# SamsungSAILMontreal/ghn3

Measured on AMD Instinct MI355X. Metric: predicted-params/sec (GHN fwd+bwd), ghn3xlm16, 256-node graphs, higher is better.
Workload: dtype f16; 1 GPU; ghn3xlm16 fwd+bwd, 1 synthetic 256-node graph(s) per GPU (seed 256000+), 86515016 predicted params per GPU, loss = sum of Frobenius norms of the predicted tensors; ghn_params=654365312, decoder_rows=1421, workspace_bytes=2436048640, zero_fill_bytes=2797339192, parallelism=dp1, index_mode=reference, loss=fused into the tile kernels

## Files before the change

ghn3_amd/build.py:

```python
import os
import subprocess
import sys
from concurrent.futures import ThreadPoolExecutor

HERE = os.path.dirname(os.path.abspath(__file__))
ROOT = os.path.dirname(HERE)
CSRC = os.path.join(HERE, 'csrc')
OUT_DIR = os.path.join(HERE, 'lib')
LIB = os.path.join(OUT_DIR, 'libghn3_hip.so')
SOURCES = ['gemm.hip', 'gemm_p8.hip', 'gemm_small.hip', 'gemm_x3.hip', 'gemm_x3d.hip', 'gemm_wg.hip', 'attention.hip', 'elementwise.hip', 'target_ops.hip', 'tnet_msa.hip', 'tnet_attn.hip', 'tnet_head.hip', 'tnet_wgrad.hip', 'tnet_join.hip', 'runtime.hip']
FLAGS = ['--offload-arch=gfx950', '-O3', '-std=c++17', '-fPIC', '-I' + os.path.join(ROOT, 'include'),
         '-I' + CSRC, '-Wno-unused-result'] + os.environ.get('GHN3_HIPCC_EXTRA', '').split()


def _hipcc():
    for cand in (os.environ.get('HIPCC'), '/opt/rocm/bin/hipcc', 'hipcc'):
        if cand and (os.path.isabs(cand) and os.path.exists(cand) or not os.path.isabs(cand)):
            return cand
    raise RuntimeError('hipcc not found')


def _stale(target, deps):
    if not os.path.exists(target):
        return True
    t = os.path.getmtime(target)
    return any(os.path.getmtime(d) > t for d in deps)


def source_hash():
    import hashlib
    h = hashlib.sha256()
    files = [os.path.join(CSRC, f) for f in sorted(os.listdir(CSRC)) if f.endswith(('.hip', '.h'))]
    files += [os.path.join(ROOT, 'include', 'ghn3_hip.h'), os.path.join(HERE, 'program.py')]
    for f in files:
        with open(f, 'rb') as fh:
            h.update(os.path.basename(f).encode() + b'\0' + fh.read())
    return h.hexdigest()[:16]


def build(force=False, verbose=True):
    os.makedirs(OUT_DIR, exist_ok=True)
    hipcc = _hipcc()
    headers = [os.path.join(ROOT, 'include', 'ghn3_hip.h'), os.path.join(CSRC, 'ghn3_internal.h'),
# ... 27 lines not shown
```

ghn3_amd/csrc/ghn3_internal.h:

```cpp
#pragma once
#include <hip/hip_runtime.h>
#include <stdint.h>
#include "ghn3_hip.h"

struct GemmProbDev {
    const float* A; const float* B; float* C;
    const float* bias; const float* residual; const float* aux_in; float* aux_out;
    const int* a_gather; const int* b_gather; const int* c_gather;
    int M, N, K, lda, ldb, ldc;
    int a_q, a_s, b_q, b_s, c_q, c_s;
    int bias_q, bias_s, bias_stride;
    int act, dact, flags;
    float alpha;
    int tile_start;
    int tiles_m, tiles_n;
    int ksplit, k_chunk;
    int order;
    int kq, ks;
    const int* lim;
    int lim_kind;
    int xcd_cols;
    int pin;
    int pin_first, pin_count;
    int pin_end, pin_total;
    const float* alpha_amax;
    int ln_kind;
    float ln_eps;
    const float* ln_p[6];
    const void* B2;
    const int* mtab;
};


int ghn3_gemm_init();
int ghn3_gemm_launch(const GemmProbDev* d_probs, int n_probs, int total_tiles, int a_mode, int b_mode,
                     int tile, int ctype, hipStream_t stream);

int ghn3_gemm_h16d_launch(const GemmProbDev* d_probs, int n_probs, int total_tiles, int tile, int ctype, int grid_cap,
                          hipStream_t stream);
int ghn3_gemm_p8_init();
int ghn3_gemm_p8_launch(const GemmProbDev* d_probs, int n_probs, int total_tiles, int ctype, int grid_cap,
                        hipStream_t stream);
int ghn3_gemm_p8w_launch(const GemmProbDev* d_probs, int n_probs, int total_tiles, int ctype, int grid_cap,
                         hipStream_t stream);
int ghn3_gemm_p8d_launch(const GemmProbDev* d_probs, int n_probs, int total_tiles, int ctype, int grid_cap,
                         hipStream_t stream);
int ghn3_gemm_x3_init();
int ghn3_gemm_x3_tile(int code, int slice, int* bm, int* bn);
int ghn3_gemm_x3_launch(const GemmProbDev* d_probs, int n_probs, int total_tiles, int code, int slice,
                        hipStream_t stream);
int ghn3_gemm_x3s_init();
int ghn3_gemm_x3s_tile(int code, int K, int ln_kind, int* bm, int* bn);
int ghn3_gemm_x3s_launch(const GemmProbDev* d_probs, const GemmProbDev* h_probs, int n_probs, int total_tiles, int code, int K,
                         int ln_kind, hipStream_t stream);
int ghn3_gemm_wg_launch(const GemmProbDev* d_probs, int n_probs, int total_tiles, int grid_cap, int tile_edge, hipStream_t stream);
int ghn3_gemm_small_launch(const GemmProbDev* d_probs, int n_probs, int total_tiles, int a_mode, int b_mode, int with_ln,
                           hipStream_t stream);

int ghn3_attn_init();
int ghn3_attn_fwd(float* out, const float* qkv, const float* bias, float* P, const int* n_nodes,
                  int B, int N, int C, int H, hipStream_t s);
int ghn3_attn_bwd(float* dqkv, const float* dO, const float* qkv, const float* P, const float* O, float* amax_out,
                  float* dBias, const int* n_nodes, int B, int N, int C, int H, int general, hipStream_t s);

int ghn3_graph_prologue(const int64_t* A, int* deg_in, int* deg_out, int* dist0, int* pair,
                        int B, int N, int V, hipStream_t s);
int ghn3_embed_nodes(float* x, const int* node_type, const int* shape_idx, const int* n_nodes, const int* node_off,
                     const float* E_type, const float* E_ch, const float* E_sp, const float* E_in,
                     const float* E_out, const float* E_dist, const int* deg_in, const int* deg_out,
                     const int* dist0, int B, int N, int C, hipStream_t s);
int ghn3_embed_bwd(const float* dx, const int* node_type, const int* shape_idx, const int* n_nodes,
                   const int* node_off, float* dE_type, float* dE_ch, float* dE_sp, float* dE_in, float* dE_out,
                   float* dE_dist, const int* deg_in, const int* deg_out, const int* dist0,
                   int B, int N, int C, int n_type, int n_ch, int n_sp, hipStream_t s);
int ghn3_edge_hidden(float* hid, const float* Pfw, const float* Pbw, int V, int C, hipStream_t s);
int ghn3_edge_hidden_bwd(float* dPfw, float* dPbw, float* dhid, const float* hid, int V, int C, hipStream_t s);
int ghn3_bias_gather(float* bias, const float* T, const int* pair, int B, int N, int H, hipStream_t s);
int ghn3_bias_hist(float* dT, const float* dBias, const int* pair, int B, int N, int H, int V, void* scratch,
                   int have_amax, hipStream_t s);
int ghn3_rowset_colsum(float* out, const float* X, const void* sets, int n_sets, int O, int I, hipStream_t s);
int ghn3_layernorm_fwd(float* y, float* x, const float* g, const float* b, float* mean, float* rstd, const float* add,
                       int n_add, int64_t add_stride, int rows, int C, float eps, hipStream_t s);
int ghn3_layernorm_bwd(float* dx, float* dy, const float* x, const float* g, const float* mean,
                       const float* rstd, const float* res, const float* add, int n_add, int64_t add_stride, int rows,
                       int C, hipStream_t s);
int ghn3_ln_param_grad(float* dg, float* db, const float* dy, const float* x, const float* mean,
                       const float* rstd, int rows, int C, int accum, hipStream_t s);
int ghn3_ln_param_grad_batch(float* gbase, const float* abase, const int64_t* table, int n_items, int rows, int C,
// ... 62 lines not shown
```

ghn3_amd/csrc/runtime.hip:

```cpp

#include "ghn3_internal.h"
#include <cstdarg>
#include <cstdio>
#include <cstring>
#include <vector>
#include <algorithm>

static thread_local char g_err[512] = "";

void ghn3_set_error(const char* fmt, ...) {
    va_list ap;
    va_start(ap, fmt);
    vsnprintf(g_err, sizeof(g_err), fmt, ap);
    va_end(ap);
}

extern "C" const char* ghn3_last_error(void) { return g_err; }
extern "C" int ghn3_abi_version(void) { return GHN3_ABI_VERSION; }

#define HIPCHK(expr)                                                                  \
    do {                                                                              \
        hipError_t e_ = (expr);                                                       \
        if (e_ != hipSuccess) {                                                       \
            ghn3_set_error("%s failed: %s", #expr, hipGetErrorString(e_));            \
// ... 161 lines not shown
        if (ms256) ms256[i] = c->tag_ms[i];
        if (n256) n256[i] = c->tag_n[i];
        if (reset) { c->tag_ms[i] = 0; c->tag_n[i] = 0; }
    }
    return GHN3_OK;
}

struct Resolver {
    void* const* bufs; int n_bufs; bool bad;
    template <typename T> T* get(const ghn3_ref& r) {
        if (r.buf < 0) return nullptr;
        if (r.buf >= n_bufs || bufs[r.buf] == nullptr) { bad = true; return nullptr; }
        return reinterpret_cast<T*>(reinterpret_cast<char*>(bufs[r.buf]) + r.off);
    }
};

static int pick_tile(const ghn3_gemm_problem& p, int forced, int64_t op_t64) {
    if (p.flags & GHN3_GEMM_X3) {
        if (forced == 44 || forced == 45 || p.ln_kind)
            return (forced == 45 ? 7000 : 6000) + 100 * (p.ln_kind & 3) + ((p.K / 64) % 100);
        return 4000 + 10 * (((forced >= 40 && forced <= 42) ? forced : 40) - 40) + p.x3_slice / 64;
    }
    if (p.ln_kind) return 32;
    if (p.flags & GHN3_GEMM_OP16) {
        if (forced == 16 || forced == 24 || forced == 20 || forced == 25 || forced == 29 || forced == 30) return forced;
        if (forced == 28) {
            const bool kmap_ok = p.b_kq == 0 || p.b_kq % 64 == 0 || 64 % p.b_kq == 0;
            return (p.ksplit <= 1 && p.M >= 160 && (p.N & 3) == 0 && kmap_ok && p.a_gather.buf < 0 && p.b_gather.buf < 0 &&
                    p.c_gather.buf < 0) ? 28 : 16;
        }
        const int64_t t256 = (int64_t)((p.M + 255) / 256) * ((p.N + 255) / 256) * (p.ksplit > 1 ? p.ksplit : 1);
        const double eff = ((double)p.M / (((p.M + 255) / 256) * 256.0)) * ((double)p.N / (((p.N + 255) / 256) * 256.0));
        return (t256 >= 200 && eff >= 0.8) ? 24 : 16;
    }
    if (forced == 48 || forced == 49) {
        const bool ok = p.a_mode == GHN3_MODE_COL && p.b_mode == GHN3_MODE_COL && p.ksplit <= 1 && (p.M & 3) == 0 &&
                        (p.N & 3) == 0 && (p.ldc & 3) == 0 && (p.C.off & 15) == 0 && (p.lda & 3) == 0 && (p.ldb & 3) == 0 &&
                        (p.A.off & 15) == 0 && (p.B.off & 15) == 0 && p.a_gather.buf < 0 &&
                        p.b_gather.buf < 0 && p.c_gather.buf < 0 && !p.a_q && !p.b_q && !p.c_q && !p.bias_q &&
                        p.act == GHN3_ACT_NONE && p.dact == GHN3_DACT_NONE && p.residual.buf < 0 && p.aux_out.buf < 0 &&
                        (p.bias.buf < 0 || (p.flags & GHN3_GEMM_BIASGRAD));
        return ok ? forced : 64;
    }
    if (forced == 32 || forced == 64 || forced == 128) return forced;
    const double flops = 2.0 * p.M * p.N * (double)p.K;
    if (p.ksplit <= 1 && op_t64 <= 640 && flops <= 4e9 && p.K <= 8192) return 32;
    const int64_t t128 = (int64_t)((p.M + 127) / 128) * ((p.N + 127) / 128) * (p.ksplit > 1 ? p.ksplit : 1);
    if (p.M >= 96 && p.N >= 96 && t128 >= 192) return 128;
    return 64;
}

static inline bool is16(int tl) { return tl == 16 || tl == 24 || tl == 20 || tl == 25 || tl == 28 || tl == 29 || tl == 30; }

extern "C" int ghn3_run(ghn3_ctx* c, const ghn3_op* ops, int n_ops, const ghn3_gemm_problem* problems, int n_problems,
                        void* const* bufs, int n_bufs, void* stream_) {
    if (!c) return GHN3_E_NOCTX;
    if (n_ops < 0 || (n_ops > 0 && !ops) || n_bufs < 0) { ghn3_set_error("ghn3_run: bad arguments"); return GHN3_E_ARG; }
    hipStream_t stream = (hipStream_t)stream_;
    Resolver R{bufs, n_bufs, false};

    std::vector<std::vector<Launch>> fresh_launches;
    const std::vector<std::vector<Launch>>* launches = &fresh_launches;
    size_t need = 0;
    for (int k = 0; k < n_ops; ++k)
        if (ops[k].kind == GHN3_OP_GEMM) need += (size_t)ops[k].i[1];
    GemmProbDev* hs = nullptr; GemmProbDev* ds = nullptr;
// ... 24 lines not shown
        for (int i = 1; i < kStageSlots; ++i)
            if (c->cache[i].stamp < c->cache[slot].stamp) slot = i;
        c->cache[slot].valid = false;
        c->cache_misses++;
        if (c->ev_used[slot]) { HIPCHK(hipEventSynchronize(c->ev[slot])); c->ev_used[slot] = false; }
        hs = c->h_stage[slot]; ds = c->d_stage[slot];
        std::vector<std::vector<Launch>>& op_launches = fresh_launches;
        op_launches.resize(n_ops);
        size_t pos = 0;
        for (int k = 0; k < n_ops; ++k) {
            if (ops[k].kind != GHN3_OP_GEMM) continue;
            const int first = (int)ops[k].i[0], cnt = (int)ops[k].i[1], forced = (int)ops[k].i[2];
            if (first < 0 || cnt < 0 || first + cnt > n_problems) {
                ghn3_set_error("op %d: GEMM problem range [%d,%d) outside table of %d", k, first, first + cnt, n_problems);
                return GHN3_E_ARG;
            }
            int64_t op_t64 = 0;
            for (int q = first; q < first + cnt; ++q)
                op_t64 += (int64_t)((problems[q].M + 63) / 64) * ((problems[q].N + 63) / 64);
            std::vector<int> codes;
            for (int q = first; q < first + cnt; ++q) {
                if (problems[q].M <= 0 || problems[q].N <= 0) continue;
                const int tc = pick_tile(problems[q], forced, op_t64);
                if (std::find(codes.begin(), codes.end(), tc) == codes.end()) codes.push_back(tc);
            }
            std::sort(codes.begin(), codes.end());
            for (int am = 0; am < 2; ++am)
                for (int bm = 0; bm < 2; ++bm)
                    for (int tl : codes) {
                        Launch L{am, bm, tl, (int)pos, 0, 0, 0, 0};
                        int te = tl == 16 ? 128 : (tl == 24 || tl == 20 || tl == 25 || tl == 28 || tl == 29 || tl == 30) ? 256 : tl == 48 ? 64 : tl == 49 ? 128 : tl;
                        int te_n = (tl == 20 || tl == 30) ? 128 : te;
                        const bool x3 = tl >= 4000;
                        const bool x3old = x3 && tl < 5000;
                        if (x3old && !ghn3_gemm_x3_tile(40 + (tl - 4000) / 10, 64 * (tl % 10), &te, &te_n)) {
                            ghn3_set_error("op %d: no split-bf16 kernel for tile bucket %d (tile code %d, K slice %d)", k, tl,
                                           40 + (tl - 4000) / 10, 64 * (tl % 10));
                            return GHN3_E_LIMIT;
                        }
                        const int x3s_code = tl >= 7000 ? 45 : 44, x3s_ln = (tl / 100) % 10, x3s_k = 64 * (tl % 100);
                        if (tl >= 6000 && !ghn3_gemm_x3s_tile(x3s_code, x3s_k, x3s_ln, &te, &te_n)) {
                            ghn3_set_error("op %d: no staged split-bf16 kernel for tile code %d, K = %d, ln_kind %d "
                                           "(gemm_x3d.hip: K = C <= 384 with a prologue; 16 x 32 tiles also K = 3C / 4C)", k,
                                           x3s_code, x3s_k, x3s_ln);
                            return GHN3_E_LIMIT;
                        }
                        std::vector<int> members, pinned_m;
                        for (int q = first; q < first + cnt; ++q) {
                            const ghn3_gemm_problem& p = problems[q];
                            if (p.M <= 0 || p.N <= 0) continue;
                            if (p.a_mode != am || p.b_mode != bm || pick_tile(p, forced, op_t64) != tl) continue;
                            members.push_back(q);
                        }
                        const bool pin_ok = (tl == 16 || tl == 20 || tl == 28) && members.size() >= 8;
                        if (pin_ok) {
                            for (int x = 0; x < 8; ++x)
                                for (int q : members)
                                    if (problems[q].xcd_pin == x + 1 && problems[q].ksplit <= 1) pinned_m.push_back(q);
                            if (!pinned_m.empty()) {
                                std::vector<int> rest;
                                for (int q : members)
                                    if (!(problems[q].xcd_pin >= 1 && problems[q].xcd_pin <= 8 && problems[q].ksplit <= 1))
                                        rest.push_back(q);
                                members = pinned_m;
                                members.insert(members.end(), rest.begin(), rest.end());
                            }
// ... 73 lines not shown
                                return GHN3_E_ARG;
                            }
                            if (p.M >= (1 << 24) || p.N >= (1 << 24) || p.K >= (1 << 24)) {
                                ghn3_set_error("op %d problem %d: M, N, K must be below 2^24", k, q);
                                return GHN3_E_LIMIT;
                            }
                            if (p.K < 0 || (p.lda & 3) || (p.ldb & 3) || (p.A.off & 15) || (p.B.off & 15)) {
                                ghn3_set_error("op %d problem %d: operands must be 16-byte aligned with ld %% 4 == 0 "
                                               "(lda=%d ldb=%d)", k, q, p.lda, p.ldb);
                                return GHN3_E_ARG;
                            }
                            GemmProbDev& g = hs[pos++];
                            g.A = R.get<const float>(p.A); g.B = R.get<const float>(p.B); g.C = R.get<float>(p.C);
                            g.bias = R.get<const float>(p.bias); g.residual = R.get<const float>(p.residual);
                            g.aux_in = R.get<const float>(p.aux_in); g.aux_out = R.get<float>(p.aux_out);
                            g.a_gather = R.get<const int>(p.a_gather); g.b_gather = R.get<const int>(p.b_gather);
                            g.c_gather = R.get<const int>(p.c_gather);
                            g.M = p.M; g.N = p.N; g.K = p.K; g.lda = p.lda; g.ldb = p.ldb; g.ldc = p.ldc;
                            g.a_q = p.a_q; g.a_s = p.a_s; g.b_q = p.b_q; g.b_s = p.b_s; g.c_q = p.c_q; g.c_s = p.c_s;
                            g.bias_q = p.bias_q; g.bias_s = p.bias_s; g.bias_stride = p.bias_stride ? p.bias_stride : 1;
                            g.act = p.act; g.dact = p.dact; g.flags = p.flags; g.alpha = p.alpha;
                            if ((p.flags & GHN3_GEMM_BIASGRAD) && (p.a_mode != GHN3_MODE_COL || !g.bias)) {
                                ghn3_set_error("op %d problem %d: BIASGRAD needs a COL-mode A and a bias ref", k, q);
                                return GHN3_E_ARG;
                            }
                            if (!g.A || !g.B || !g.C || (p.dact != GHN3_DACT_NONE && !g.aux_in)) {
                                ghn3_set_error("op %d problem %d: missing A/B/C/aux_in buffer", k, q);
                                return GHN3_E_ARG;
                            }
                            g.tile_start = L.tiles;
                            g.tiles_m = (p.M + te - 1) / te;
                            g.tiles_n = (p.N + te_n - 1) / te_n;
                            g.mtab = nullptr;
                            if (tl == 28 && p.mtiles.buf >= 0) {
                                g.mtab = R.get<const int>(p.mtiles);
                                g.tiles_m = p.n_mtiles;
                            }
                            g.pin = pin_x + 1; g.pin_first = g.pin_count = 0;
                            g.pin_end = pin_end; g.pin_total = n_pinned;
                            if (pin_x >= 0) {
                                g.tile_start = pin_local[pin_x];
                                pin_local[pin_x] += g.tiles_m * g.tiles_n;
                                if (pin_count[pin_x]++ == 0) pin_first[pin_x] = member_i;
                            }
                            g.kq = is16(tl) ? p.b_kq : 0; g.ks = p.b_ks;
                            g.lim = is16(tl) ? R.get<const int>(p.lim) : nullptr;
                            g.lim_kind = (g.lim || (tl == 28 && p.mtiles.buf >= 0)) ? p.lim_kind : 0;
                            g.alpha_amax = is16(tl) ? R.get<const float>(p.alpha_amax) : nullptr;
                            g.B2 = x3 ? R.get<const void>(p.B2) : nullptr;
                            if (x3old && p.x3_slice > L.max_slice) L.max_slice = p.x3_slice;
                            if (x3 && !x3old) L.max_slice = p.K;
                            g.ln_kind = p.ln_kind; g.ln_eps = p.ln_eps;
                            if (p.ln_kind) L.with_ln = 1;
                            for (int e = 0; e < 6; ++e) g.ln_p[e] = p.ln_kind ? R.get<const float>(p.ln_p[e]) : nullptr;
                            if (p.ln_kind) {
                                const bool ok = (p.ln_kind == 1 || p.ln_kind == 2) && p.a_mode == GHN3_MODE_ROW &&
                                                p.a_gather.buf < 0 && p.a_q == 0 && p.K <= 4096 && (p.K & 3) == 0 &&
                                                !(p.flags & GHN3_GEMM_OP16) && g.ln_p[0] &&
                                                (p.ln_kind == 1 ? g.ln_p[1] != nullptr
                                                                : (g.ln_p[1] && g.ln_p[2] && g.ln_p[3]));
                                if (!ok) {
                                    ghn3_set_error("op %d problem %d: the LayerNorm row prologue needs a ROW-mode fp32 A "
                                                   "without gather, K %% 4 == 0, K <= 4096 and its parameter refs", k, q);
                                    return GHN3_E_ARG;
                                }
                            }
                            g.order = (int64_t)p.M > (int64_t)p.N ? 1 : 0;
                            if (tl == 28) g.order = 0;
                            g.ksplit = p.ksplit > 1 ? p.ksplit : 1;
                            g.k_chunk = x3old ? p.x3_slice : x3 ? p.K : ((p.K + g.ksplit - 1) / g.ksplit + 63) / 64 * 64;
                            if (g.ksplit > 1 && (p.bias.buf >= 0 || p.act || p.dact || p.residual.buf >= 0 ||
                                                 p.aux_out.buf >= 0)) {
                                ghn3_set_error("op %d problem %d: split-K allows no epilogue but alpha", k, q);
                                return GHN3_E_ARG;
                            }
                            g.xcd_cols = 0;
                            if (pin_x >= 0) {
                            } else if (tl == 25 || tl == 29 || tl == 30) {
                                static const int64_t b_budget = getenv("GHN3_XCD_B_BYTES") ? atoll(getenv("GHN3_XCD_B_BYTES"))
                                                                                          : (int64_t)(5 << 19);
                                int G = 1;
                                while (G < 8 && (int64_t)p.N * p.K * 2 / G > b_budget && g.tiles_n >= 2 * G) G *= 2;
                                g.xcd_cols = G;
                                const int npg = (g.tiles_n + G - 1) / G, mpc = (g.tiles_m + 8 / G - 1) / (8 / G);
                                L.tiles += 8 * npg * mpc;
                            } else if (tl == 32 || tl == 48 || tl == 49 || x3) {
                                L.tiles += g.tiles_m * g.tiles_n;
                            } else {
                                const int per_split = g.order ? ((g.tiles_m + 7) / 8 * 8) * g.tiles_n
                                                              : g.tiles_m * ((g.tiles_n + 7) / 8 * 8);
                                L.tiles += per_split * g.ksplit;
                            }
                            L.count++;
                        }
                        if (n_pinned)
                            for (int x = 0; x < 8; ++x) {
                                hs[L.first + x].pin_first = pin_first[x];
                                hs[L.first + x].pin_count = pin_count[x];
                            }
                        if (L.count > 0) op_launches[k].push_back(L);
                    }
        }
        if (R.bad) { ghn3_set_error("ghn3_run: a GEMM problem references an absent buffer"); return GHN3_E_ARG; }
        HIPCHK(hipMemcpyAsync(ds, hs, pos * sizeof(GemmProbDev), hipMemcpyHostToDevice, stream));
        HIPCHK(hipEventRecord(c->ev[slot], stream));
        c->ev_used[slot] = true;
        if (use_cache) {
            SlotCache& e = c->cache[slot];
            e.n_ops = n_ops; e.n_problems = n_problems; e.n_bufs = n_bufs;
            e.ops.assign(ops, ops + n_ops);
            e.problems.assign(problems, problems + n_problems);
            e.bufs.assign(bufs, bufs + n_bufs);
            e.launches.swap(fresh_launches);
            launches = &e.launches;
            e.up_stream = stream;
            e.stamp = ++c->clock;
            e.valid = true;
        } else {
            c->cache[slot].stamp = ++c->clock;
// ... 44 lines not shown
                HIPCHK(hipEventRecord(c->ev_fork, main_stream));
                HIPCHK(hipStreamWaitEvent(c->side, c->ev_fork, 0));
                main_dirty = false;
            }
            side_dirty = true;
        } else {
            main_dirty = true;
        }
        hipStream_t stream = on_side ? c->side : main_stream;
        const bool timed = (c->profile == 2 || c->profile == 3) && (o.flags & GHN3_OPFLAG_TIMED);
        if (c->profile == 1) HIPCHK(hipEventRecord(c->pe0, stream));
        if (timed) {
            if (c->pool_used >= 8192) { int rc2 = drain_pool(c); if (rc2) return rc2; }
            if (c->pool->size() < 2 * (c->pool_used + 1)) {
                hipEvent_t e0, e1;
                HIPCHK(hipEventCreate(&e0));
                HIPCHK(hipEventCreate(&e1));
                c->pool->push_back(e0); c->pool->push_back(e1);
                c->pool_tag->push_back(0);
            }
            (*c->pool_tag)[c->pool_used] = (o.flags >> 16) & 255;
            HIPCHK(hipEventRecord((*c->pool)[2 * c->pool_used], stream));
        }
        switch (o.kind) {
        case GHN3_OP_NOP: break;
        case GHN3_OP_GEMM:
            for (const Launch& L : (*launches)[k]) {
                if (L.tile >= 6000)
                    rc = ghn3_gemm_x3s_launch(ds + L.first, hs + L.first, L.count, L.tiles, L.tile >= 7000 ? 45 : 44, L.max_slice,
                                              (L.tile / 100) % 10, stream);
                else if (L.tile >= 4000)
                    rc = ghn3_gemm_x3_launch(ds + L.first, L.count, L.tiles, 40 + (L.tile - 4000) / 10,
                                             64 * (L.tile % 10), stream);
                else if (L.tile == 48 || L.tile == 49)
                    rc = ghn3_gemm_wg_launch(ds + L.first, L.count, L.tiles, gemm_cap, L.tile == 49 ? 128 : 64, stream);
                else if (L.tile == 32)
                    rc = ghn3_gemm_small_launch(ds + L.first, L.count, L.tiles, L.a_mode, L.b_mode, L.with_ln, stream);
                else if (L.tile == 30)
                    rc = ghn3_gemm_p8d_launch(ds + L.first, L.count, L.tiles,
                                              (o.flags & 0xff) ? ((o.flags & 0xff) - 1) : c->ctype, gemm_cap, stream);
                else if (L.tile == 29)
                    rc = ghn3_gemm_p8w_launch(ds + L.first, L.count, L.tiles,
                                              (o.flags & 0xff) ? ((o.flags & 0xff) - 1) : c->ctype, gemm_cap, stream);
                else if (L.tile == 28)
                    rc = ghn3_gemm_p8_launch(ds + L.first, L.count, L.tiles,
                                             (o.flags & 0xff) ? ((o.flags & 0xff) - 1) : c->ctype, gemm_cap, stream);
                else if (is16(L.tile))
                    rc = ghn3_gemm_h16d_launch(ds + L.first, L.count, L.tiles,
                                               L.tile == 16 ? 128 : L.tile == 20 ? 20 : L.tile == 25 ? 25 : 256,
                                               (o.flags & 0xff) ? ((o.flags & 0xff) - 1) : c->ctype, gemm_cap,
                                               stream);
                else
                    rc = ghn3_gemm_launch(ds + L.first, L.count, L.tiles, L.a_mode, L.b_mode, L.tile,
                                          (o.flags & 0xff) ? ((o.flags & 0xff) - 1) : c->ctype, stream);
                if (rc) break;
            }
            break;
        case GHN3_OP_GRAPH_PROLOGUE:
            rc = ghn3_graph_prologue(R.get<const int64_t>(o.r[0]), R.get<int>(o.r[1]), R.get<int>(o.r[2]),
                                     R.get<int>(o.r[3]), R.get<int>(o.r[4]), (int)o.i[0], (int)o.i[1], (int)o.i[2],
                                     stream);
            break;
        case GHN3_OP_EMBED_NODES:
            rc = ghn3_embed_nodes(R.get<float>(o.r[0]), R.get<const int>(o.r[1]), R.get<const int>(o.r[2]),
                                  R.get<const int>(o.r[3]), R.get<const int>(o.r[4]), R.get<const float>(o.r[5]),
                                  R.get<const float>(o.r[6]), R.get<const float>(o.r[7]), R.get<const float>(o.r[8]),
// ... 235 lines not shown
```

ghn3_amd/program.py:

```python

import math
import os

import numpy as np

from . import _lib as L
from . import bookkeeping as bk

ALIGN = 256


def global_param_names():
    return ['ln.weight', 'ln.bias', 'embed.weight', 'shape_enc.embed_spatial.weight',
            'shape_enc.embed_channel.weight', 'gnn.0.centrality_embed_in.weight',
            'gnn.0.centrality_embed_out.weight', 'gnn.0.input_dist_embed.weight',
            'gnn.0.attn.edge_embed.embed.weight', 'gnn.0.attn.proj_e.0.weight', 'gnn.0.attn.proj_e.0.bias',
            'gnn.0.attn.proj_e.2.weight', 'gnn.0.attn.proj_e.2.bias',
            'decoder.fc.0.weight', 'decoder.fc.0.bias', 'decoder.conv.0.weight', 'decoder.conv.0.bias',
            'decoder.conv.2.weight', 'decoder.conv.2.bias', 'decoder.class_layer_predictor.1.weight',
            'decoder.class_layer_predictor.1.bias', 'decoder_1d.fc.0.weight', 'decoder_1d.fc.0.bias',
            'decoder_1d.fc.2.weight', 'decoder_1d.fc.2.bias', 'bias_class.1.weight', 'bias_class.1.bias']


LAYER_PARAM_NAMES = ['ln1.weight', 'ln1.bias', 'attn.to_qkv.weight', 'attn.to_out.0.weight', 'attn.to_out.0.bias',
# ... 4 lines not shown
def param_names(layers, layernorm=True):
    names = global_param_names()
    if not layernorm:
        names = [n for n in names if not n.startswith('ln.')]
    for l in range(layers):
        names += ['gnn.%d.%s' % (l, n) for n in LAYER_PARAM_NAMES]
    return names


def round_up(x, m):
    return (x + m - 1) // m * m


class Program:

    X_WS, X_IDX, X_EDGES, X_OUT, X_DOUT, X_TOK, X_SCAL, X_GRADFLAT, X_SHADOW, X_NORMG, X_COUNT = range(11)

    def __init__(self, cfg, node_infos, n_nodes, node_types, max_edge, nets, index_mode='reference',
                 training=True, predict_class_layers=True, reduce_graph=False, layernorm=True, weight_norm=True,
                 decoder_ctype=None, decoder_bwd_ctype=None, direct16=True, side_stream=True, graphormer_x3=None):
        self.cfg = cfg
        self.SIDE = L.OPFLAG_SIDE if side_stream else 0
        self.split_k2 = os.environ.get('GHN3_SPLIT_K2', '1') != '0'
        self.split_k2_min = int(os.environ.get('GHN3_SPLIT_K2_MIN', '768'))
        self.decoder_ctype = decoder_ctype
        if decoder_bwd_ctype is None:
            decoder_bwd_ctype = decoder_ctype
        self.decoder_bwd_ctype = decoder_bwd_ctype
        self.bwd_scaled = decoder_bwd_ctype == L.CT_F16
        self.direct16 = bool(direct16) and decoder_ctype in (L.CT_F16, L.CT_BF16) and (8 * int(cfg['hid'])) % 64 == 0
        self.d12_fwd_ctype = {'f32': L.CT_F32, 'f16': None}[os.environ.get('GHN3_D12_FWD', 'f32')]
        self.use_p8 = os.environ.get('GHN3_P8', '1') != '0'
        self.d1_bwd_ctype = {'f32': L.CT_F32, 'f16': None}[os.environ.get('GHN3_D1_BWD', 'f32')]
        self.C = C = int(cfg['hid'])
        if graphormer_x3 is None:
            graphormer_x3 = decoder_ctype in (L.CT_F16, L.CT_BF16) and os.environ.get('GHN3_X3', '1') != '0'
        self.x3 = bool(graphormer_x3) and C % 64 == 0 and 64 <= C <= 384
        self.x3s = self.x3 and C in (64, 128, 256, 384) and os.environ.get('GHN3_X3S', '1') != '0'
        self.x3f16 = self.x3s and os.environ.get('GHN3_X3_F16', '1') != '0'
        self.H = int(cfg['heads'])
        self.Lyr = int(cfg['layers'])
        self.K = int(cfg['num_classes'])
        self.max_shape = tuple(int(v) for v in cfg['max_shape'])
        self.S = self.max_shape[2]
        assert self.max_shape[2] == self.max_shape[3]
        self.layernorm = layernorm
        self.weight_norm = weight_norm
        self.training = training
        self.index_mode = index_mode
        self.names = param_names(self.Lyr, layernorm)
        self.P = len(self.names)
        self.slot = {n: i for i, n in enumerate(self.names)}
        self.B = len(n_nodes)
        self.n_nodes = [int(v) for v in n_nodes]
        self.N = max(self.n_nodes)
        self.V = int(max_edge) + 1
        if self.V + 1 > 257:
            raise ValueError('shortest-path length %d exceeds the 257-row edge embedding (graphormer.py:95-96)'
                             % max_edge)
        if self.N > 4096:
            raise ValueError('graphs with more than 4096 nodes are not supported (got %d)' % self.N)
        self._ops, self._probs, self._ln = [], [], {}
        self.tag_flops = {}
        self._ws = 0
        self._ws_names = {}
        self._idx_chunks, self._idx_size = [], 0
# ... 871 lines not shown
            p0 = self.gemm(xe, self.pref(W1), h1d, self.n1, 2 * C, C, C, C, 2 * C, bias=self.pref(b1),
                           act=L.ACT_RELU, a_gather=r_src1)
            self.gemm_op(p0)
            p0 = len(self._probs)
            if self.n1_plain:
                self.gemm(h1d, self.pref(W2d), w1d, self.n1_plain, 2 * mc, 2 * C, 2 * C, 2 * C, 2 * mc,
                          bias=self.pref(b2d))
            if self.n1_clsb:
                self.gemm(self.wref('h1d', self.n1_plain * 2 * C), self.pref(W2d),
                          self.wref('w1d', self.n1_plain * 2 * mc), self.n1_clsb, 2 * mc, 2 * C, 2 * C, 2 * C, 2 * mc,
                          bias=self.pref(b2d), act=L.ACT_RELU)
            self.gemm_op(p0)
            if self.n1_clsb:
                cbout = self.wsf('cbout', self.n1_clsb * ldK)
                p0 = self.gemm(self.wref('w1d', self.n1_plain * 2 * mc + mc), self.pref(Wb), cbout, self.n1_clsb, K,
                               mc, 2 * mc, mc, ldK, bias=self.pref(bb))
                self.gemm_op(p0)

        if self.SIDE:
            self.op(L.OP_JOIN)
        if M > 0:
            t = self.wsf('t', M * 4 * C)
            u = self.wsf('u', M * 8 * C)
            self.d1 = []
            p0 = len(self._probs)
            for p in np.unique(self.row_pos):
                rws = np.nonzero(self.row_pos == p)[0].astype(np.int32)
                r_rows = self.idx(rws)
                r_src = self.idx(self.row_src[rws])
                self.d1.append((int(p), len(rws), r_rows, r_src))
                self.gemm(xe, self.pref(Wfc, int(p) * C), t, len(rws), 4 * C, C, C, S2 * C, 4 * C,
                          bias=self.pref(bfc, int(p)), bias_stride=S2, act=L.ACT_RELU, a_gather=r_src,
                          c_gather=r_rows)
            self.gemm_op(p0, tag=self.TAG_D1_FWD, ctype=self.d12_fwd_ctype)
            d2_fix = self.decoder_ctype in (L.CT_F16, L.CT_BF16) and os.environ.get('GHN3_D2_FIX', '1') != '0' and \
                self.d12_fwd_ctype == L.CT_F32
            p0 = self.gemm(t, self.pref(W0), u, M, 8 * C, 4 * C, 4 * C, 4 * C, 8 * C, bias=self.pref(b0),
                           act=L.ACT_NONE if d2_fix else L.ACT_RELU)
            self.gemm_op(p0, tag=self.TAG_D2_FWD, ctype=self.decoder_ctype if d2_fix else self.d12_fwd_ctype)
            if d2_fix:
                self.op(L.OP_RELU_FIX, refs=(u, t, self.pref(W0), self.pref(b0)),
                        ints=(M, 8 * C, 8 * C, 4 * C, 0, 0),
                        floats=(float(os.environ.get('GHN3_RELU_FIX_TAU', '5e-3')),))
            p0 = len(self._probs)
            tiles_floats = 0
            for gg in self.gemm_groups:
                gg['tile_off'] = tiles_floats
                for g in gg['members']:
                    g['tile_off'] = tiles_floats + (g['row0'] - gg['row0']) * gg['ld']
                tiles_floats += round_up(gg['rows'] * gg['ld'], 64)
            for g in self.conv_groups:
                if 'resize' in g:
                    g['rs_off'] = tiles_floats
                    tiles_floats += round_up(g['resize'][0] * g['resize'][1] * g['ld'], 64)
            self.tiles_floats = tiles_floats
            tiles = self.wsf('tiles', tiles_floats)
            use16 = any(g['op16'] for g in self.gemm_groups)
            if use16:
                fct = self.decoder_ctype
                self.op(L.OP_JOIN)
                self.uh = self.ws16('uh', M * 8 * C)
                self.cast16((self.xbuf(self.X_WS), 0),
                            [dict(src_off=u[1] // 4, rows=M, cols=8 * C, ld_src=8 * C, straight=(self.uh, 8 * C, fct))])
            fl = 0.0
            for g in self.gemm_groups:
                fl += sum(2.0 * sb['rows'] * sb['cols'] * 8 * C for sb in g['subs'])
                if g['op16'] and g['p8'] and self.P8_BALANCED:
# ... 815 lines not shown
                               accum=True, op16=True, alpha_amax=amax_u)
                self.gemm_op(p0, ctype=bct, tag=self.TAG_D2_BWD, side=True, flops=2.0 * 8 * C * 4 * C * M)
                d2_tile = int(os.environ.get('GHN3_D2_DGRAD_TILE', '0'))
                ks = int(os.environ.get('GHN3_D2_DGRAD_KS', '0')) or \
                    max(1, min(4, 320 // max(1, ((M + 127) // 128) * ((4 * C + 127) // 128))))
                while ks > 1 and (8 * C) % (64 * ks):
                    ks -= 1
                if ks > 1:
                    kc = 8 * C // ks
                    planes = self.wsf('d_t_parts', (ks - 1) * M * 4 * C)
                    p0 = len(self._probs)
                    for j in range(ks):
                        dst = d_t if j == 0 else (planes[0], planes[1] + 4 * (j - 1) * M * 4 * C)
                        self.gemm(self.href(duh + j * kc), self.sref(self.w0hT + j * kc), dst, M, 4 * C, kc, 8 * C, 8 * C,
                                  4 * C, op16=True, alpha_amax=amax_u)
                    self.gemm_op(p0, ctype=bct, tag=self.TAG_D2_BWD, flops=2.0 * M * 4 * C * 8 * C, tile=d2_tile)
                    self.op(L.OP_DACT, refs=(d_t, t, self.NONE, planes),
                            ints=(M, 4 * C, 4 * C, L.DACT_RELU, ks - 1, M * 4 * C, M))
                else:
                    p0 = self.gemm(self.href(duh), self.sref(self.w0hT), d_t, M, 4 * C, 8 * C, 8 * C, 8 * C, 4 * C,
                                   dact=L.DACT_RELU, aux_in=t, op16=True, alpha_amax=amax_u)
                    self.gemm_op(p0, ctype=bct, tag=self.TAG_D2_BWD)
            else:
                p0 = self.gemm(d_u, t, self.gref(W0), 8 * C, 4 * C, M, 8 * C, 4 * C, 4 * C, a_mode=L.MODE_COL,
                               b_mode=L.MODE_COL, accum=True, dbias=self.gref(b0))
                self.gemm_op(p0, tag=self.TAG_D2_BWD, side=True)
                p0 = self.gemm(d_u, self.pref(W0), d_t, M, 4 * C, 8 * C, 8 * C, 4 * C, 4 * C, a_mode=L.MODE_ROW,
                               b_mode=L.MODE_COL, dact=L.DACT_RELU, aux_in=t)
                self.gemm_op(p0, tag=self.TAG_D2_BWD)
            p0 = len(self._probs)
            for (p, cnt, r_rows, r_src) in self.d1:
                self.gemm(d_t, self.pref(Wfc, p * C), d_rows, cnt, C, 4 * C, 4 * C, S2 * C, C, a_mode=L.MODE_ROW,
                          b_mode=L.MODE_COL, a_gather=r_rows, c_gather=r_rows)
            self.gemm_op(p0, tag=self.TAG_D1_BWD, ctype=self.d1_bwd_ctype, tile=int(os.environ.get('GHN3_D1_DGRAD_TILE', '0')))
            p0 = len(self._probs)
            for (p, cnt, r_rows, r_src) in self.d1:
                self.gemm(d_t, xe, self.gref(Wfc, p * C), 4 * C, C, cnt, 4 * C, C, S2 * C, a_mode=L.MODE_COL,
                          b_mode=L.MODE_COL, a_gather=r_rows, b_gather=r_src, accum=True,
                          dbias=self.gref(bfc, p), dbias_stride=S2)
            self.gemm_op(p0, tag=self.TAG_D1_BWD, side=True, ctype=self.d1_bwd_ctype)
        if not early_1d:
            decoder_1d_bwd(False)
        self.bwd_split = len(self._ops)
        all_src = np.concatenate([self.row_src, self.oned_src]) if (M + n1) else np.zeros(0, dtype=np.int32)
        order = np.argsort(all_src, kind='stable').astype(np.int32)
        counts = np.bincount(all_src, minlength=rows)[:rows]
        seg_ptr = np.concatenate([[0], np.cumsum(counts)]).astype(np.int32)
        d_xe = self.wsf('d_xe', rows * C)
        if early_1d:
            self.op(L.OP_JOIN, ints=(2, 0))
        self.op(L.OP_ROWSEG_SUM, refs=(d_xe, d_rows, self.idx(seg_ptr), self.idx(order)), ints=(rows, C, C, C, 0))

        dxa = self.wsf('dxa', rows * C)
        do = self.wsf('do', rows * C)
        nb_ = round_up(4 * B * H * N * N, 16)
        dBias = self.wsf('dBias', nb_ // 4 + 2 * V * V * H + 16)
        hist = (dBias[0], dBias[1] + nb_)
        hist_amax = (dBias[0], dBias[1] + nb_ + 8 * V * V * H)
        self.op(L.OP_MEMSET0, refs=(dBias,), ints=(nb_ + 8 * V * V * H + 16,))
        xL = self.wref('x%d' % self.Lyr)
        if self.layernorm:
            self.op(L.OP_LAYERNORM_BWD, refs=(dxa, d_xe, xL, self.pref('ln.weight'), self.wref('mf'), self.wref('rf'),
                                              self.NONE), ints=(rows, C))
            self.op(L.OP_LN_PARAM_GRAD, refs=(self.gref('ln.weight'), self.gref('ln.bias'), d_xe, xL,
                                              self.wref('mf'), self.wref('rf')), ints=(rows, C, 1), flags=self.SIDE)
            g_cur = dxa
        else:
            g_cur = d_xe
        bias = self.wref('bias')
        pending_ln1 = None
        side_group = max(1, int(os.environ.get('GHN3_SIDE_GROUP', '4'))) if self.SIDE else 1
        side_pending = []
        layer_side = []
# ... 119 lines not shown
```

Measured before the change: 15.30 billion predicted-params/s.

## Add register-resident-weight fp32 MFMA kernels for decoder fc fwd, dgrad and wgrad

Adds a new gemm_fc kernel family for the decoder's first fc layer, which has a small K (at most a few hundred). The forward and dgrad kernels keep a slice of the weights in registers and stream gathered activation rows through fp32 MFMA. Wgrad writes the reduction over rows directly, with no split-K. Tile code 52 routes the D1 forward, dgrad and wgrad gemms to these kernels by default, and wgrad now overwrites instead of accumulating. The goal is to avoid padded-tile overhead and launch cost of the generic gemm paths for these thin, gathered problems; the risks are limited parallelism (one block per N slice) and correctness if the weight-gradient buffer was meant to be accumulated.

```diff
diff --git a/ghn3_amd/build.py b/ghn3_amd/build.py
--- a/ghn3_amd/build.py
+++ b/ghn3_amd/build.py
@@ -8,7 +8,7 @@
 CSRC = os.path.join(HERE, 'csrc')
 OUT_DIR = os.path.join(HERE, 'lib')
 LIB = os.path.join(OUT_DIR, 'libghn3_hip.so')
-SOURCES = ['gemm.hip', 'gemm_p8.hip', 'gemm_small.hip', 'gemm_x3.hip', 'gemm_x3d.hip', 'gemm_wg.hip', 'attention.hip', 'elementwise.hip', 'target_ops.hip', 'tnet_msa.hip', 'tnet_attn.hip', 'tnet_head.hip', 'tnet_wgrad.hip', 'tnet_join.hip', 'runtime.hip']
+SOURCES = ['gemm.hip', 'gemm_p8.hip', 'gemm_small.hip', 'gemm_x3.hip', 'gemm_x3d.hip', 'gemm_wg.hip', 'gemm_fc.hip', 'attention.hip', 'elementwise.hip', 'target_ops.hip', 'tnet_msa.hip', 'tnet_attn.hip', 'tnet_head.hip', 'tnet_wgrad.hip', 'tnet_join.hip', 'runtime.hip']
 FLAGS = ['--offload-arch=gfx950', '-O3', '-std=c++17', '-fPIC', '-I' + os.path.join(ROOT, 'include'),
          '-I' + CSRC, '-Wno-unused-result'] + os.environ.get('GHN3_HIPCC_EXTRA', '').split()
 
diff --git a/ghn3_amd/csrc/gemm_fc.hip b/ghn3_amd/csrc/gemm_fc.hip
--- /dev/null
+++ b/ghn3_amd/csrc/gemm_fc.hip
@@ -0,0 +1,291 @@
+
+#include "ghn3_internal.h"
+
+#define GAS __attribute__((address_space(1)))
+typedef float f32x4 __attribute__((ext_vector_type(4)));
+typedef float f32x2 __attribute__((ext_vector_type(2)));
+typedef f32x4 GAS* gf4;
+typedef const f32x4 GAS* gcf4;
+typedef const f32x2 GAS* gcf2;
+typedef const int GAS* gci;
+
+namespace {
+
+__device__ __forceinline__ const GemmProbDev* fc_find(const GemmProbDev* __restrict__ probs, int n_probs, int tile) {
+    int lo = 0, hi = n_probs - 1;
+    while (lo < hi) {
+        const int mid = (lo + hi + 1) >> 1;
+        if (probs[mid].tile_start <= tile) lo = mid; else hi = mid - 1;
+    }
+    return probs + lo;
+}
+
+constexpr int FC_RB = 512;
+
+template <int KQ>
+__global__ __launch_bounds__(256, 2) void fc_fwd_kernel(const GemmProbDev* __restrict__ probs, int n_probs) {
+    constexpr int KS = 4 * KQ;
+    const GemmProbDev* P = fc_find(probs, n_probs, blockIdx.x);
+    const int lane = threadIdx.x & 63, wave = threadIdx.x >> 6, i16 = lane & 15, q = lane >> 4;
+    const int M = P->M, N = P->N;
+    const int nb = (blockIdx.x - P->tile_start) * 64 + wave * 16;
+    const bool active = nb < N;
+    const f32x4 zero = f32x4{0.f, 0.f, 0.f, 0.f};
+    __shared__ int s_src[FC_RB], s_dst[FC_RB];
+
+    const int wn = min(nb + i16, N - 1);
+    const float GAS* wrow = (const float GAS*)P->B + (int64_t)wn * P->ldb + 4 * q;
+    f32x4 w[KS];
+#pragma unroll
+    for (int s = 0; s < KS; ++s) w[s] = active ? *reinterpret_cast<gcf4>(wrow + 16 * s) : zero;
+
+    const int n = nb + 4 * q;
+    const bool n_ok = n < N;
+    f32x4 bias = zero;
+    if (P->bias && n_ok) {
+        const float GAS* bp = (const float GAS*)P->bias;
+#pragma unroll
+        for (int e = 0; e < 4; ++e) bias[e] = bp[(int64_t)(n + e) * P->bias_stride];
+    }
+    const float alpha = P->alpha;
+    const bool relu = P->act == GHN3_ACT_RELU, accum = (P->flags & GHN3_GEMM_ACCUM) != 0;
+    const float GAS* Ag = (const float GAS*)P->A;
+    float GAS* Cg = (float GAS*)P->C;
+    gci ag = (gci)P->a_gather;
+    gci cg = (gci)P->c_gather;
+    const int lda = P->lda, ldc = P->ldc;
+    constexpr int KH = KS / 2;
+
+    for (int mb = 0; mb < M; mb += FC_RB) {
+        const int rows = min(FC_RB, M - mb);
+        if (mb) __syncthreads();
+        for (int i = threadIdx.x; i < rows; i += 256) {
+            s_src[i] = ag ? ag[mb + i] : mb + i;
+            s_dst[i] = cg ? cg[mb + i] : mb + i;
+        }
+        __syncthreads();
+        if (!active) continue;
+        f32x4 a0[KH], a1[KH];
+        const float GAS* arow = Ag + (int64_t)s_src[min(i16, rows - 1)] * lda + 4 * q;
+#pragma unroll
+        for (int s = 0; s < KH; ++s) a0[s] = *reinterpret_cast<gcf4>(arow + 16 * s);
+#pragma unroll
+        for (int s = 0; s < KH; ++s) a1[s] = *reinterpret_cast<gcf4>(arow + 16 * (KH + s));
+        for (int m0 = 0; m0 < rows; m0 += 16) {
+            const int m = m0 + i16;
+            arow = Ag + (int64_t)s_src[min(m + 16, rows - 1)] * lda + 4 * q;
+            f32x4 acc = zero;
+#pragma unroll
+            for (int s = 0; s < KH; ++s)
+#pragma unroll
+                for (int j = 0; j < 4; ++j) acc = __builtin_amdgcn_mfma_f32_16x16x4f32(w[s][j], a0[s][j], acc, 0, 0, 0);
+            __builtin_amdgcn_sched_barrier(0);
+#pragma unroll
+            for (int s = 0; s < KH; ++s) a0[s] = *reinterpret_cast<gcf4>(arow + 16 * s);
+            __builtin_amdgcn_sched_barrier(0);
+#pragma unroll
+            for (int s = 0; s < KH; ++s)
+#pragma unroll
+                for (int j = 0; j < 4; ++j) acc = __builtin_amdgcn_mfma_f32_16x16x4f32(w[KH + s][j], a1[s][j], acc, 0, 0, 0);
+            __builtin_amdgcn_sched_barrier(0);
+#pragma unroll
+            for (int s = 0; s < KH; ++s) a1[s] = *reinterpret_cast<gcf4>(arow + 16 * (KH + s));
+            if (m < rows && n_ok) {
+                f32x4 v = acc * alpha + bias;
+                if (relu) {
+#pragma unroll
+                    for (int e = 0; e < 4; ++e) v[e] = fmaxf(v[e], 0.f);
+                }
+                float GAS* dst = Cg + (int64_t)s_dst[m] * ldc + n;
+                if (accum) v += *reinterpret_cast<gcf4>(dst);
+                *reinterpret_cast<gf4>(dst) = v;
+            }
+        }
+    }
+}
+
+constexpr int FCD_LD = 36;
+
+template <int KD>
+__global__ __launch_bounds__(512, 4) void fc_dgrad_kernel(const GemmProbDev* __restrict__ probs, int n_probs) {
+    constexpr int NS = 2 * KD;
+    __shared__ __attribute__((aligned(16))) float red[8 * 16 * FCD_LD];
+    const GemmProbDev* P = fc_find(probs, n_probs, blockIdx.x);
+    const int tid = threadIdx.x, lane = tid & 63, wave = tid >> 6, i16 = lane & 15, q = lane >> 4;
+    const int M = P->M, N = P->N;
+    const int nb = (blockIdx.x - P->tile_start) * 32;
+    const int kw = wave * NS * 16;
+    const f32x4 zero = f32x4{0.f, 0.f, 0.f, 0.f};
+
+    const int wc = nb + 2 * i16;
+    const bool w_ok = wc < N;
+    const float GAS* wp = (const float GAS*)P->B + (int64_t)(kw + 4 * q) * P->ldb + (w_ok ? wc : 0);
+    const int64_t ldb = P->ldb;
+    f32x2 w[NS][4];
+#pragma unroll
+    for (int t = 0; t < NS; ++t)
+#pragma unroll
+        for (int j = 0; j < 4; ++j) {
+            const f32x2 v = *reinterpret_cast<gcf2>(wp + (16 * t + j) * ldb);
+            w[t][j] = w_ok ? v : f32x2{0.f, 0.f};
+        }
+
+    const float alpha = P->alpha;
+    const bool accum = (P->flags & GHN3_GEMM_ACCUM) != 0;
+    const float GAS* Ag = (const float GAS*)P->A;
+    float GAS* Cg = (float GAS*)P->C;
+    gci ag = (gci)P->a_gather;
+    gci cg = (gci)P->c_gather;
+    const int lda = P->lda, ldc = P->ldc;
+    float* mine = red + (wave * 16 + i16) * FCD_LD + 8 * q;
+    const int rr = tid >> 5, rc = tid & 31;
+
+    for (int m0 = 0; m0 < M; m0 += 16) {
+        const int mr = min(m0 + i16, M - 1);
+        const float GAS* arow = Ag + (int64_t)(ag ? ag[mr] : mr) * lda + kw + 4 * q;
+        f32x4 acc0 = zero, acc1 = zero;
+#pragma unroll
+        for (int t = 0; t < NS; ++t) {
+            const f32x4 a = *reinterpret_cast<gcf4>(arow + 16 * t);
+#pragma unroll
+            for (int j = 0; j < 4; ++j) {
+                acc0 = __builtin_amdgcn_mfma_f32_16x16x4f32(w[t][j][0], a[j], acc0, 0, 0, 0);
+                acc1 = __builtin_amdgcn_mfma_f32_16x16x4f32(w[t][j][1], a[j], acc1, 0, 0, 0);
+            }
+        }
+        *reinterpret_cast<f32x4*>(mine) = f32x4{acc0[0], acc1[0], acc0[1], acc1[1]};
+        *reinterpret_cast<f32x4*>(mine + 4) = f32x4{acc0[2], acc1[2], acc0[3], acc1[3]};
+        __syncthreads();
+        float s = red[rr * FCD_LD + rc];
+#pragma unroll
+        for (int v = 1; v < 8; ++v) s += red[(v * 16 + rr) * FCD_LD + rc];
+        const int m = m0 + rr;
+        if (m < M && nb + rc < N) {
+            float GAS* dst = Cg + (int64_t)(cg ? cg[m] : m) * ldc + nb + rc;
+            s *= alpha;
+            if (accum) s += *dst;
+            *dst = s;
+        }
+        __syncthreads();
+    }
+}
+
+__global__ __launch_bounds__(384, 4) void fc_wgrad_kernel(const GemmProbDev* __restrict__ probs, int n_probs) {
+    const GemmProbDev* P = fc_find(probs, n_probs, blockIdx.x);
+    const int lane = threadIdx.x & 63, wave = threadIdx.x >> 6, n_waves = blockDim.x >> 6, i16 = lane & 15, q = lane >> 4;
+    const int M = P->M, N = P->N, K = P->K;
+    const int m0 = (blockIdx.x - P->tile_start) * 32;
+    const f32x4 zero = f32x4{0.f, 0.f, 0.f, 0.f};
+    const f32x2 zero2 = f32x2{0.f, 0.f};
+    const float GAS* Ag = (const float GAS*)P->A;
+    const float GAS* Bg = (const float GAS*)P->B;
+    float GAS* Cg = (float GAS*)P->C;
+    gci ga = (gci)P->a_gather;
+    gci gb = (gci)P->b_gather;
+    const int lda = P->lda, ldb = P->ldb, ldc = P->ldc;
+    const float alpha = P->alpha;
+    const bool accum = (P->flags & GHN3_GEMM_ACCUM) != 0;
+    const int ma = m0 + 2 * i16;
+    const bool a_ok = ma < M;
+
+    for (int nt = wave; nt * 64 < N; nt += n_waves) {
+        const int nbn = nt * 64 + 4 * i16;
+        const bool b_ok = nbn < N;
+        f32x4 acc[2][4];
+#pragma unroll
+        for (int j = 0; j < 2; ++j)
+#pragma unroll
+            for (int jj = 0; jj < 4; ++jj) acc[j][jj] = zero;
+        f32x2 bsum = zero2;
+        int ia[4], ib[4];
+#pragma unroll
+        for (int u = 0; u < 4; ++u) {
+            const int k = min(4 * u + q, K - 1);
+            ia[u] = ga ? ga[k] : k;
+            ib[u] = gb ? gb[k] : k;
+        }
+        for (int k0 = 0; k0 < K; k0 += 16) {
+            f32x2 a[4];
+            f32x4 b[4];
+#pragma unroll
+            for (int u = 0; u < 4; ++u) {
+                const bool k_ok = k0 + 4 * u + q < K;
+                a[u] = (k_ok && a_ok) ? *reinterpret_cast<gcf2>(Ag + (int64_t)ia[u] * lda + ma) : zero2;
+                b[u] = (k_ok && b_ok) ? *reinterpret_cast<gcf4>(Bg + (int64_t)ib[u] * ldb + nbn) : zero;
+            }
+#pragma unroll
+            for (int u = 0; u < 4; ++u) {
+                const int k = min(k0 + 16 + 4 * u + q, K - 1);
+                ia[u] = ga ? ga[k] : k;
+                ib[u] = gb ? gb[k] : k;
+            }
+#pragma unroll
+            for (int u = 0; u < 4; ++u) {
+                bsum += a[u];
+#pragma unroll
+                for (int j = 0; j < 2; ++j)
+#pragma unroll
+                    for (int jj = 0; jj < 4; ++jj)
+                        acc[j][jj] = __builtin_amdgcn_mfma_f32_16x16x4f32(a[u][j], b[u][jj], acc[j][jj], 0, 0, 0);
+            }
+        }
+        if (b_ok) {
+#pragma unroll
+            for (int r = 0; r < 4; ++r)
+#pragma unroll
+                for (int j = 0; j < 2; ++j) {
+                    const int m = m0 + 2 * (4 * q + r) + j;
+                    if (m >= M) continue;
+                    float GAS* dst = Cg + (int64_t)m * ldc + nbn;
+                    f32x4 v = f32x4{acc[j][0][r], acc[j][1][r], acc[j][2][r], acc[j][3][r]} * alpha;
+                    if (accum) v += *reinterpret_cast<gcf4>(dst);
+                    *reinterpret_cast<gf4>(dst) = v;
+                }
+        }
+        if (nt == 0 && (P->flags & GHN3_GEMM_BIASGRAD)) {
+#pragma unroll
+            for (int e = 0; e < 2; ++e) {
+                float t = bsum[e];
+                t += __shfl_xor(t, 16, 64);
+                t += __shfl_xor(t, 32, 64);
+                bsum[e] = t;
+            }
+            if (q == 0 && a_ok) {
+                float GAS* db = (float GAS*)P->bias;
+#pragma unroll
+                for (int e = 0; e < 2; ++e) db[(int64_t)(ma + e) * P->bias_stride] += bsum[e];
+            }
+        }
+    }
+}
+
+template <int KQ>
+void fc_fwd_go(const GemmProbDev* d_probs, int n_probs, int total_tiles, hipStream_t stream) {
+    hipLaunchKernelGGL(fc_fwd_kernel<KQ>, dim3(total_tiles), dim3(256), 0, stream, d_probs, n_probs);
+}
+template <int KD>
+void fc_dgrad_go(const GemmProbDev* d_probs, int n_probs, int total_tiles, hipStream_t stream) {
+    hipLaunchKernelGGL(fc_dgrad_kernel<KD>, dim3(total_tiles), dim3(512), 0, stream, d_probs, n_probs);
+}
+
+}
+
+int ghn3_gemm_fc_launch(const GemmProbDev* d_probs, int n_probs, int total_tiles, int a_mode, int b_mode, int k_idx, int max_n,
+                        hipStream_t stream) {
+    if (n_probs <= 0 || total_tiles <= 0) return GHN3_OK;
+    if (a_mode == GHN3_MODE_COL && b_mode == GHN3_MODE_COL) {
+        const int waves = max_n >= 384 ? 6 : max_n > 64 ? (max_n + 63) / 64 : 1;
+        hipLaunchKernelGGL(fc_wgrad_kernel, dim3(total_tiles), dim3(64 * waves), 0, stream, d_probs, n_probs);
+    } else if (a_mode == GHN3_MODE_ROW && k_idx >= 1 && k_idx <= 6) {
+        typedef void (*go_t)(const GemmProbDev*, int, int, hipStream_t);
+        static const go_t fwd[6] = {fc_fwd_go<1>, fc_fwd_go<2>, fc_fwd_go<3>, fc_fwd_go<4>, fc_fwd_go<5>, fc_fwd_go<6>};
+        static const go_t dgrad[6] = {fc_dgrad_go<1>, fc_dgrad_go<2>, fc_dgrad_go<3>, fc_dgrad_go<4>, fc_dgrad_go<5>, fc_dgrad_go<6>};
+        (b_mode == GHN3_MODE_ROW ? fwd : dgrad)[k_idx - 1](d_probs, n_probs, total_tiles, stream);
+    } else {
+        ghn3_set_error("fc stream gemm: no kernel for modes %d / %d, K index %d", a_mode, b_mode, k_idx);
+        return GHN3_E_ARG;
+    }
+    hipError_t e = hipGetLastError();
+    if (e != hipSuccess) { ghn3_set_error("fc stream gemm launch: %s", hipGetErrorString(e)); return GHN3_E_HIP; }
+    return GHN3_OK;
+}
diff --git a/ghn3_amd/csrc/ghn3_internal.h b/ghn3_amd/csrc/ghn3_internal.h
--- a/ghn3_amd/csrc/ghn3_internal.h
+++ b/ghn3_amd/csrc/ghn3_internal.h
@@ -54,6 +54,8 @@
 int ghn3_gemm_x3s_launch(const GemmProbDev* d_probs, const GemmProbDev* h_probs, int n_probs, int total_tiles, int code, int K,
                          int ln_kind, hipStream_t stream);
 int ghn3_gemm_wg_launch(const GemmProbDev* d_probs, int n_probs, int total_tiles, int grid_cap, int tile_edge, hipStream_t stream);
+int ghn3_gemm_fc_launch(const GemmProbDev* d_probs, int n_probs, int total_tiles, int a_mode, int b_mode, int k_idx, int max_n,
+                        hipStream_t stream);
 int ghn3_gemm_small_launch(const GemmProbDev* d_probs, int n_probs, int total_tiles, int a_mode, int b_mode, int with_ln,
                            hipStream_t stream);
 
diff --git a/ghn3_amd/csrc/runtime.hip b/ghn3_amd/csrc/runtime.hip
--- a/ghn3_amd/csrc/runtime.hip
+++ b/ghn3_amd/csrc/runtime.hip
@@ -217,6 +217,26 @@
         const int64_t t256 = (int64_t)((p.M + 255) / 256) * ((p.N + 255) / 256) * (p.ksplit > 1 ? p.ksplit : 1);
         const double eff = ((double)p.M / (((p.M + 255) / 256) * 256.0)) * ((double)p.N / (((p.N + 255) / 256) * 256.0));
         return (t256 >= 200 && eff >= 0.8) ? 24 : 16;
+    }
+    if (forced == 52) {
+        bool ok = p.ksplit <= 1 && (p.N & 3) == 0 && (p.lda & 3) == 0 && (p.ldb & 3) == 0 && (p.ldc & 3) == 0 &&
+                  (p.A.off & 15) == 0 && (p.B.off & 15) == 0 && (p.C.off & 15) == 0 && !p.a_q && !p.b_q && !p.c_q && !p.bias_q &&
+                  p.residual.buf < 0 && p.aux_out.buf < 0 && p.aux_in.buf < 0 && p.dact == GHN3_DACT_NONE && p.K >= 1;
+        int idx = 0;
+        if (p.a_mode == GHN3_MODE_ROW && p.b_mode == GHN3_MODE_ROW) {
+            ok = ok && p.K % 64 == 0 && p.K <= 384 && p.b_gather.buf < 0 && !(p.flags & GHN3_GEMM_BIASGRAD) &&
+                 (p.act == GHN3_ACT_NONE || p.act == GHN3_ACT_RELU);
+            idx = p.K / 64;
+        } else if (p.a_mode == GHN3_MODE_ROW && p.b_mode == GHN3_MODE_COL) {
+            ok = ok && p.K % 256 == 0 && p.K <= 1536 && p.b_gather.buf < 0 && p.bias.buf < 0 && p.act == GHN3_ACT_NONE;
+            idx = p.K / 256;
+        } else if (p.a_mode == GHN3_MODE_COL && p.b_mode == GHN3_MODE_COL) {
+            ok = ok && (p.M & 3) == 0 && p.c_gather.buf < 0 && p.act == GHN3_ACT_NONE &&
+                 (p.bias.buf < 0 || (p.flags & GHN3_GEMM_BIASGRAD));
+        } else {
+            ok = false;
+        }
+        return ok ? 520 + idx : pick_tile(p, 0, op_t64);
     }
     if (forced == 48 || forced == 49) {
         const bool ok = p.a_mode == GHN3_MODE_COL && p.b_mode == GHN3_MODE_COL && p.ksplit <= 1 && (p.M & 3) == 0 &&
@@ -307,6 +327,7 @@
                         int te = tl == 16 ? 128 : (tl == 24 || tl == 20 || tl == 25 || tl == 28 || tl == 29 || tl == 30) ? 256 : tl == 48 ? 64 : tl == 49 ? 128 : tl;
                         int te_n = (tl == 20 || tl == 30) ? 128 : te;
                         const bool x3 = tl >= 4000;
+                        const bool fc = tl >= 520 && tl < 530;
                         const bool x3old = x3 && tl < 5000;
                         if (x3old && !ghn3_gemm_x3_tile(40 + (tl - 4000) / 10, 64 * (tl % 10), &te, &te_n)) {
                             ghn3_set_error("op %d: no split-bf16 kernel for tile bucket %d (tile code %d, K slice %d)", k, tl,
@@ -446,6 +467,12 @@
                             g.tiles_m = (p.M + te - 1) / te;
                             g.tiles_n = (p.N + te_n - 1) / te_n;
                             g.mtab = nullptr;
+                            if (fc) {
+                                const bool wgrad = p.a_mode == GHN3_MODE_COL;
+                                g.tiles_m = wgrad ? (p.M + 31) / 32 : 1;
+                                g.tiles_n = wgrad ? 1 : p.b_mode == GHN3_MODE_ROW ? (p.N + 63) / 64 : (p.N + 31) / 32;
+                                if (p.N > L.max_slice) L.max_slice = p.N;
+                            }
                             if (tl == 28 && p.mtiles.buf >= 0) {
                                 g.mtab = R.get<const int>(p.mtiles);
                                 g.tiles_m = p.n_mtiles;
@@ -498,7 +525,7 @@
                                 g.xcd_cols = G;
                                 const int npg = (g.tiles_n + G - 1) / G, mpc = (g.tiles_m + 8 / G - 1) / (8 / G);
                                 L.tiles += 8 * npg * mpc;
-                            } else if (tl == 32 || tl == 48 || tl == 49 || x3) {
+                            } else if (tl == 32 || tl == 48 || tl == 49 || x3 || fc) {
                                 L.tiles += g.tiles_m * g.tiles_n;
                             } else {
                                 const int per_split = g.order ? ((g.tiles_m + 7) / 8 * 8) * g.tiles_n
@@ -609,6 +636,8 @@
                 else if (L.tile >= 4000)
                     rc = ghn3_gemm_x3_launch(ds + L.first, L.count, L.tiles, 40 + (L.tile - 4000) / 10,
                                              64 * (L.tile % 10), stream);
+                else if (L.tile >= 520 && L.tile < 530)
+                    rc = ghn3_gemm_fc_launch(ds + L.first, L.count, L.tiles, L.a_mode, L.b_mode, L.tile - 520, L.max_slice, stream);
                 else if (L.tile == 48 || L.tile == 49)
                     rc = ghn3_gemm_wg_launch(ds + L.first, L.count, L.tiles, gemm_cap, L.tile == 49 ? 128 : 64, stream);
                 else if (L.tile == 32)
diff --git a/ghn3_amd/program.py b/ghn3_amd/program.py
--- a/ghn3_amd/program.py
+++ b/ghn3_amd/program.py
@@ -60,6 +60,7 @@
         self.d12_fwd_ctype = {'f32': L.CT_F32, 'f16': None}[os.environ.get('GHN3_D12_FWD', 'f32')]
         self.use_p8 = os.environ.get('GHN3_P8', '1') != '0'
         self.d1_bwd_ctype = {'f32': L.CT_F32, 'f16': None}[os.environ.get('GHN3_D1_BWD', 'f32')]
+        self.fc_stream = os.environ.get('GHN3_FC_STREAM', '1') != '0'
         self.C = C = int(cfg['hid'])
         if graphormer_x3 is None:
             graphormer_x3 = decoder_ctype in (L.CT_F16, L.CT_BF16) and os.environ.get('GHN3_X3', '1') != '0'
@@ -997,7 +998,8 @@
                 self.gemm(xe, self.pref(Wfc, int(p) * C), t, len(rws), 4 * C, C, C, S2 * C, 4 * C,
                           bias=self.pref(bfc, int(p)), bias_stride=S2, act=L.ACT_RELU, a_gather=r_src,
                           c_gather=r_rows)
-            self.gemm_op(p0, tag=self.TAG_D1_FWD, ctype=self.d12_fwd_ctype)
+            self.gemm_op(p0, tag=self.TAG_D1_FWD, ctype=self.d12_fwd_ctype,
+                         tile=52 if self.fc_stream and self.d12_fwd_ctype == L.CT_F32 else 0)
             d2_fix = self.decoder_ctype in (L.CT_F16, L.CT_BF16) and os.environ.get('GHN3_D2_FIX', '1') != '0' and \
                 self.d12_fwd_ctype == L.CT_F32
             p0 = self.gemm(t, self.pref(W0), u, M, 8 * C, 4 * C, 4 * C, 4 * C, 8 * C, bias=self.pref(b0),
@@ -1879,13 +1881,15 @@
             for (p, cnt, r_rows, r_src) in self.d1:
                 self.gemm(d_t, self.pref(Wfc, p * C), d_rows, cnt, C, 4 * C, 4 * C, S2 * C, C, a_mode=L.MODE_ROW,
                           b_mode=L.MODE_COL, a_gather=r_rows, c_gather=r_rows)
-            self.gemm_op(p0, tag=self.TAG_D1_BWD, ctype=self.d1_bwd_ctype, tile=int(os.environ.get('GHN3_D1_DGRAD_TILE', '0')))
+            fc_tile = 52 if self.fc_stream and self.d1_bwd_ctype == L.CT_F32 else 0
+            self.gemm_op(p0, tag=self.TAG_D1_BWD, ctype=self.d1_bwd_ctype,
+                         tile=int(os.environ.get('GHN3_D1_DGRAD_TILE', str(fc_tile))))
             p0 = len(self._probs)
             for (p, cnt, r_rows, r_src) in self.d1:
                 self.gemm(d_t, xe, self.gref(Wfc, p * C), 4 * C, C, cnt, 4 * C, C, S2 * C, a_mode=L.MODE_COL,
-                          b_mode=L.MODE_COL, a_gather=r_rows, b_gather=r_src, accum=True,
+                          b_mode=L.MODE_COL, a_gather=r_rows, b_gather=r_src, accum=not fc_tile,
                           dbias=self.gref(bfc, p), dbias_stride=S2)
-            self.gemm_op(p0, tag=self.TAG_D1_BWD, side=True, ctype=self.d1_bwd_ctype)
+            self.gemm_op(p0, tag=self.TAG_D1_BWD, side=True, ctype=self.d1_bwd_ctype, tile=fc_tile)
         if not early_1d:
             decoder_1d_bwd(False)
         self.bwd_split = len(self._ops)
```

New measurement: 15.48 billion predicted-params/s, median of 3. About the same (+1.1%).
